# tonfengerqiguyisui/mapping-private

Measured on AMD Instinct MI355X. Metric: Mvoxels/s C3-HLAC + detections/s sliding-box, 256^3 grid, higher is better.
Workload: dtype u8 x u8 -> u32 (exact integer C3-HLAC), f32 search

## Files before the change

mapping-private_amd/csrc/c3h_internal.h:

```cpp
#pragma once
#include <hip/hip_runtime.h>

#include <cstdint>
#include <cstdlib>
#include <string>
#include <mutex>
#include <vector>

#include "../../include/c3hlac_mi355x.h"

namespace c3h {

constexpr uint32_t kOcc = 1u << 24;
constexpr uint32_t kEmptyKey = 0xffffffffu;
constexpr int kBlock = 256;
constexpr int kTileMax = 16;

constexpr float kNorm0 = 1 / 255.0;
constexpr float kNorm1 = 1 / 65025.0;
constexpr float kNorm117_1 = 1 / 845325.0;
constexpr float kNorm117_1Bin = 1 / 13.0;

template <class T>
struct DevBuf {
// ... 261 lines not shown
  const int32_t* types;
  int32_t* trans;
  int div_b[3], min_b[3], off[3], sb[3];
  float leaf, inv_leaf, inv_s;
  int hist1;
};
hipError_t nbr_build(NbrGrid& g, uint32_t* keys, uint32_t* keys2, uint32_t* idx, uint32_t* idx2, void* tmp,
                     size_t* tmp_bytes, hipStream_t s);
hipError_t launch_normals(const NbrGrid& g, float radius, const float vp[3], float4* out, hipStream_t s);
hipError_t launch_rsd(const NbrGrid& g, const float4* nrm, const float4* cent, int64_t nc, float max_dist,
                      float2* radii, int32_t* types, hipStream_t s);
hipError_t launch_grsd(const GrsdArgs& a, hipStream_t s);
hipError_t launch_grsd_feat(const int32_t* trans, int64_t H, float norm, float* out, int stride, hipStream_t s);
hipError_t launch_vosch_concat(const float* grsd, const float* c3, const int32_t* exist, int64_t H, float* out,
                               hipStream_t s);
hipError_t launch_pc2_convert(const void* data, uint32_t height, uint32_t width, uint32_t point_step,
                              uint32_t row_step, const int32_t off[4], int big, float* out, hipStream_t s);
hipError_t launch_exist_rule(const float* feat, int64_t H, int dim, int rule, int32_t* exist, hipStream_t s);

hipError_t launch_compress(const float* feat, int64_t H, int F, const float* axis_pt, int D,
                           int Dpad, const float* fmax, int fmax_len, float* G,
                           const int32_t* rows, const uint32_t* nrows, const int32_t* exist,
                           hipStream_t s);
hipError_t launch_masked_rows(const float* src, const int32_t* exist, int64_t H, int W, float* dst,
                              hipStream_t s);

struct ScoreLaunch {
  const float* G;
  const int32_t* exist;
  int D;
  int xn, yn, zn;
  int xr, yr, zr;
  int xe, ye, ze;
  int thr;
  const float* axis_q;
  const float* qt;
  int M, r, Opad;
  double* scores;
  ScorePartial* partials;
  int64_t order_base;
};
hipError_t launch_score(const ScoreLaunch& a, hipStream_t s);
bool score_fast_ok(int D, int r);
int64_t score_blocks(const ScoreLaunch& a);

struct ModeGeom {
  int64_t offset;
  int64_t P;
  int xe, ye, xr, yr, zr;
  int mode;
};
struct SparseSearch {
  const float* G;
  const int32_t* exist;
  int D, xn, yn, zn, thr;
  const float* qt;
  int M, r, Opad;
  int mpg;
  int group_loop;
  double* scores;
  ModeGeom md[6];
  int nmodes;
  int64_t pstart[7];
  int64_t order_base[6];
  long long* list;
  uint32_t* cnt;
  uint32_t epoch;
  int nframes;
  int64_t s_G, s_exist, s_scores, s_list, s_cnt, s_partials, s_lists;
  c3h_det* outs[kMaxBatch];
  ScorePartial* partials;
  uint32_t* done;
  c3h_det* lists;
  int clean;
  long long* prof;
  float* gbox = nullptr;
  int64_t s_gbox = 0;
  int score_mfma = 0;
  int skip_empty = 1;
  const _Float16* qt16 = nullptr;
  int Kq16 = 0;
  const int32_t* lim = nullptr;
  int sparse_scores = 0;
};
bool score_mfma_ok(int D);
struct SparseCompress {
  const float* feat;
  const float* PT;
  const float* fmax;
  float* G;
  const int32_t* rows;
  const uint32_t* nrows;
  int F, D, Dpad, fmax_len;
  int64_t H;
  int64_t s_feat, s_G, s_rows, s_nrows;
  const _Float16* PT16 = nullptr;
  int Fp16 = 0;
  const _Float16* feat16 = nullptr;
  const uint32_t* feat16_flag = nullptr;
  int f16s = 0;
};
bool compress_rows_ok(int F, int Dpad);
constexpr int64_t kBoxsumRows = 65536;
constexpr int64_t kCompressMfmaRows = 65536;
hipError_t launch_sparse_search(const SparseSearch& a, const SparseCompress* sc, hipStream_t s);
int64_t sparse_score_blocks(const SparseSearch& a);

struct ReplayMode {
  int64_t offset;
  int64_t P;
  int xe, ye;
  int mode;
};
struct ReplayModes {
  ReplayMode m[6];
  int n;
};
hipError_t launch_replay(const double* scores, const ReplayModes& modes, int M, int rank,
                         int r1, int r2, int r3, int clean, c3h_det* lists, c3h_det* out2,
                         hipStream_t s);

hipError_t launch_clean_lists(c3h_det* lists, int n, hipStream_t s);

struct TickParts {
  const C3Launch* occ = nullptr;
  const C3Launch* tile = nullptr;
  const SparseSearch* gate = nullptr;
  const SparseCompress* comp = nullptr;
  const SparseSearch* score = nullptr;
  DevBuf<long long>* prof = nullptr;
};
bool tick_ok(const C3Launch& l);
hipError_t launch_tick(const TickParts& p, hipStream_t s);
size_t c3hlac_lds_bytes(int tw_max, int list_max);
int64_t leaf_layout_blocks(int64_t nvox);

}

struct c3h_ctx {
  int device = 0;
  hipStream_t stream = nullptr;
  hipStream_t own_stream = nullptr;
  std::string err;

  c3h_ctx* parent = nullptr;
  std::vector<c3h_ctx*> lanes;
  std::vector<hipEvent_t> lane_ev;
  hipEvent_t fork_ev = nullptr;
  int nlanes = 3;
  int nbatch = 32;
  bool pipeline = true;
  uint64_t setup_version = 0;
  std::vector<float> h_axis_p, h_var, h_axis_q, h_fmax;

  bool have_grid = false;
  c3h_grid_info info{};
  c3h::DevBuf<uint32_t> grid;
  const uint32_t* grid_ptr = nullptr;
  c3h::DevBuf<float> pts;
  c3h::DevBuf<uint32_t> raw;
  c3h::DevBuf<float> dsbuf;
  c3h::DevBuf<float4> normals;
  bool normals_valid = false;
  c3h::NbrGrid nbr{};
  c3h::DevBuf<uint32_t> nkeys, nkeys2, nidx, nidx2, ncstart, ncend;
  c3h::DevBuf<uint8_t> ntmp;
// ... 159 lines not shown
```

mapping-private_amd/csrc/capi.hip:

```cpp
#include <algorithm>
#include <climits>
#include <cmath>
#include <cstdio>
#include <cstdlib>
#include <cstring>
#include <thread>

#include "c3h_internal.h"

using c3h::DevBuf;

namespace {

int fail(c3h_ctx* ctx, int code, const std::string& msg) {
  if (ctx) ctx->err = msg;
  return code;
}
int hip_fail(c3h_ctx* ctx, const char* what, hipError_t e) {
  return fail(ctx, C3H_ERR_HIP, std::string(what) + ": " + hipGetErrorString(e));
}

#define HIPCHK(expr)                                     \
  do {                                                   \
    hipError_t e_ = (expr);                              \
// ... 2078 lines not shown

struct PipeScope {
  c3h_ctx* ctx;
  hipStream_t saved[kPipeDepth - 1];
  explicit PipeScope(c3h_ctx* c) : ctx(c) {
    ctx->pipe_busy = true;
    for (int l = 0; l < kPipeDepth - 1 && l < (int)ctx->lanes.size(); ++l) {
      saved[l] = ctx->lanes[l]->stream;
      ctx->lanes[l]->stream = ctx->stream;
    }
  }
  ~PipeScope() {
    for (int l = 0; l < kPipeDepth - 1 && l < (int)ctx->lanes.size(); ++l) ctx->lanes[l]->stream = saved[l];
    ctx->pipe_busy = false;
  }
};

int pipe_tick(c3h_ctx* ctx, const c3h_ctx::PipeBatch* fresh) {
  c3h::TickParts tp;
  tp.prof = &ctx->prof;
  if (fresh && !fresh->stamped) tp.occ = &fresh->l;
  for (auto& b : ctx->pipe) {
    if (b.age == 1) tp.tile = &b.l;
    if (b.age == 2) {
      tp.gate = &b.q;
      tp.comp = &b.sc;
    }
    if (b.age == 3) tp.score = &b.q;
  }
  {
    Timed tm(ctx, 5, fresh ? fresh->nf : 0);
    hipError_t e = c3h::launch_tick(tp, ctx->stream);
    if (e != hipSuccess) return hip_fail(ctx, "launch_tick", e);
  }
  for (auto& b : ctx->pipe) {
    if (b.age == 2 && b.set) b.set->scores_layout = b.layout;
    if (b.age == 1 && b.fix) {
      hipError_t e = c3h::launch_point_fixup(b.fx, ctx->stream);
      if (e != hipSuccess) return hip_fail(ctx, "launch_point_fixup", e);
    }
  }
  std::vector<c3h_ctx::PipeBatch> next;
  for (auto& b : ctx->pipe)
    if (b.age < 3) {
      next.push_back(b);
      next.back().age++;
    }
  if (fresh) {
    next.push_back(*fresh);
    next.back().age = 1;
  }
  ctx->pipe.swap(next);
  return C3H_OK;
}

int pipe_flush(c3h_ctx* ctx) {
  if (ctx->pipe.empty()) return C3H_OK;
  PipeScope scope(ctx);
  while (!ctx->pipe.empty()) {
    int rc = pipe_tick(ctx, nullptr);
    if (rc != C3H_OK) {
      ctx->pipe.clear();
      return rc;
    }
  }
  return C3H_OK;
}

int pipe_quiesce(c3h_ctx* ctx) {
  if (ctx->pipe_busy || ctx->pipe.empty()) return C3H_OK;
  return pipe_flush(ctx);
}

int pipe_prepare(c3h_ctx* ctx, const uint32_t* const* grids, c3h_det* const* outs, int nb,
                 const c3h_ctx::PipeKey& k, const int32_t* lim, c3h_ctx::PipeBatch* fresh) {
  c3h_ctx* c = pipe_set(ctx, ctx->pipe_seq);
  c->capture = true;
  c->cap_c3_valid = c->cap_search_valid = false;
  int rc = c3h_set_grid(c, grids[0], k.div_b, k.min_b, k.leaf, 1);
  if (rc == C3H_OK) rc = extract_frames(c, grids, nb, &k.p, nullptr, nullptr);
  if (rc == C3H_OK) rc = search_frames(c, nb, k.range, k.thr, k.rotate, outs, 2);
  c->capture = false;
  c->cap_q.lim = lim;
  if (rc < 0) {
    if (c != ctx) ctx->err = c->err;
    return rc;
  }
  const bool fits = c->cap_c3_valid && c->cap_search_valid && c->cap_sparse_g && c->cap_argmax &&
                    c3h::tick_ok(c->cap_c3);
  if (!fits) {
    if (!ctx->pipe.empty()) return fail(ctx, C3H_ERR_STATE, "pipeline: internal: geometry changed");
    return 0;
  }
  c->nframes_feat = 1;
  *fresh = c3h_ctx::PipeBatch{c->cap_c3, c->cap_q, c->cap_sc, nb, 0};
  fresh->set = c;
  fresh->layout = c->cap_layout;
  return rc;
}

int pipe_commit(c3h_ctx* ctx, const c3h_ctx::PipeBatch& fresh, const c3h_ctx::PipeKey& k, int rc) {
  if (ctx->pipe.empty()) {
    for (int sidx = 0; sidx < kPipeDepth; ++sidx) {
      c3h_ctx* c = sidx == 0 ? ctx : (sidx - 1 < (int)ctx->lanes.size() ? ctx->lanes[sidx - 1] : nullptr);
      if (c && c->tileflags.p && c->tileflags.n >= 2)
        HIPCHK(hipMemsetAsync(c->tileflags.p, 0, 2 * sizeof(uint32_t), ctx->stream));
    }
  }
  int trc = pipe_tick(ctx, &fresh);
  if (trc != C3H_OK) return trc;
  ctx->pipe_seq++;
  ctx->pipe_key = k;
  ctx->pipe_nm = rc;
  return rc;
}

int pipe_push(c3h_ctx* ctx, const uint32_t* const* grids, c3h_det* const* outs, int nb,
              const c3h_ctx::PipeKey& k, const int32_t* lim = nullptr) {
  c3h_ctx::PipeBatch fresh{};
  const int rc = pipe_prepare(ctx, grids, outs, nb, k, lim, &fresh);
  if (rc <= 0) return rc;
  return pipe_commit(ctx, fresh, k, rc);
}

c3h_ctx::PipeKey pipe_key(c3h_ctx* ctx, const int32_t div_b[3], const int32_t min_b[3], float leaf,
                          const c3h_extract_params* p, const int32_t range[3], int32_t thr, int32_t rotate,
                          int B) {
  c3h_ctx::PipeKey k;
  memset(&k, 0, sizeof(k));
  memcpy(k.div_b, div_b, sizeof(k.div_b));
  memcpy(k.min_b, min_b, sizeof(k.min_b));
  k.leaf = leaf;
  k.p = *p;
  memcpy(k.range, range, sizeof(k.range));
  k.thr = thr;
  k.rotate = rotate ? 1 : 0;
  k.batch = B;
  k.rank = ctx->rank;
  k.setup_version = ctx->setup_version;
  return k;
}

bool pipelinable(const c3h_ctx* ctx) {
  return ctx->pipeline && ctx->rank == 1 && c3h::score_fast_ok(ctx->D, ctx->r);
}

int run_frames_pipelined(c3h_ctx* ctx, const uint32_t* const* d_grids, int32_t nframes,
                         const int32_t div_b[3], const int32_t min_b[3], float leaf,
                         const c3h_extract_params* p, const int32_t range[3], int32_t exist_threshold,
                         int32_t rotate, c3h_det* d_out, int B, bool drain) {
  const size_t per_frame = (size_t)std::max(ctx->M, 1) * ctx->rank;
  const int nchunks = (nframes + B - 1) / B;
  int rc = ensure_lanes(ctx, kPipeDepth - 1);
  if (rc != C3H_OK) return rc;
  const c3h_ctx::PipeKey k = pipe_key(ctx, div_b, min_b, leaf, p, range, exist_threshold, rotate, B);
  if (!ctx->pipe.empty() && memcmp(&k, &ctx->pipe_key, sizeof(k)) != 0) {
    rc = pipe_flush(ctx);
    if (rc != C3H_OK) return rc;
  }
  PipeScope scope(ctx);
  if (drain && ctx->pipe.empty())
    ctx->pipe_seq = (uint64_t)((kPipeDepth - (nchunks - 1) % kPipeDepth) % kPipeDepth);
  int nm = 0;
  for (int ch = 0; ch < nchunks; ++ch) {
    const uint32_t* grids[c3h::kMaxBatch];
    c3h_det* outs[c3h::kMaxBatch];
// ... 686 lines not shown
```

mapping-private_amd/csrc/pipeline.hip:

```cpp
#include <algorithm>
#include <climits>
#include <cstdio>
#include <cstdlib>
#include <cstring>
#include <vector>

#include "c3hlac_dev.h"
#include "search_dev.h"

namespace c3h {
namespace {

struct TickArgs {
  int n_score, n_cg, n_tile, n_occ;
  SparseSearch sq;
  int s_gx, s_groups;
  SparseSearch gq;
  CompressRows cr;
  int g_ngate, g_ncomp;
  int comp_mfma;
  KArgs ka;
  int t_grid;
  OccArgs oa;
  int o_grid;
  int order;
  int xcd;
  long long* prof;
};

__device__ __forceinline__ int tick_canonical_block(const TickArgs& t) {
  const int n[4] = {t.n_occ, t.n_tile, t.n_cg, t.n_score};
  int b = blockIdx.x;
  for (int i = 0; i < 4; ++i) {
    const int r = (t.order >> (4 * i)) & 15;
    if (b < n[r]) {
      for (int k = 0; k < r; ++k) b += n[k];
      return b;
    }
    b -= n[r];
  }
  return b;
}

#ifndef C3H_TICK_PRIO_OCC
#define C3H_TICK_PRIO_OCC 3
#endif
#ifndef C3H_TICK_PRIO_TILE
#define C3H_TICK_PRIO_TILE 0
#endif
#ifndef C3H_TICK_PRIO_CG
#define C3H_TICK_PRIO_CG 0
#endif
#ifndef C3H_TICK_PRIO_SCORE
#define C3H_TICK_PRIO_SCORE 0
#endif
#define C3H_SETPRIO(p) \
  if constexpr ((p) > 0) __builtin_amdgcn_s_setprio(p)

__device__ __forceinline__ void role_frame(int b, int g, bool xcd, int& f, int& local) {
  if (xcd) {
    const int q = b >> 3, k = q / g;
    f = (b & 7) + 8 * k;
    local = q - k * g;
  } else {
    f = b / g;
    local = b - f * g;
  }
}

__device__ __forceinline__ void tick_roles(const TickArgs& t, uint32_t* tick_smem) {
  int b = t.order == 0x3210 ? (int)blockIdx.x : tick_canonical_block(t);
  int f, r;
  if (b < t.n_occ) {
    C3H_SETPRIO(C3H_TICK_PRIO_OCC);
    role_frame(b, t.o_grid, t.xcd & 1, f, r);
    occupancy_bits_body<true>(t.oa, r, f, t.o_grid, tick_smem);
    return;
  }
  b -= t.n_occ;
  if (b < t.n_tile) {
    C3H_SETPRIO(C3H_TICK_PRIO_TILE);
    role_frame(b, t.t_grid, t.xcd & 2, f, r);
    if (t.ka.wave117) c3hlac_wave117_body(t.ka, r, f, t.t_grid, tick_smem);
    else c3hlac_tile_body(t.ka, r, f, t.t_grid, tick_smem);
    return;
  }
  b -= t.n_tile;
  if (b < t.n_cg) {
    C3H_SETPRIO(C3H_TICK_PRIO_CG);
    role_frame(b, t.g_ngate + t.g_ncomp, t.xcd & 4, f, r);
    if (r < t.g_ngate) gate_body(t.gq, r, f);
    else if (t.comp_mfma) compress_f32t_body(t.cr, r - t.g_ngate, t.g_ncomp, f, reinterpret_cast<float*>(tick_smem));
    else compress_rows_body(t.cr, r - t.g_ngate, t.g_ncomp, f, reinterpret_cast<float*>(tick_smem));
    return;
  }
  b -= t.n_cg;
  C3H_SETPRIO(C3H_TICK_PRIO_SCORE);
  role_frame(b, t.s_gx * t.s_groups, t.xcd & 8, f, r);
  score_list_body(t.sq, r % t.s_gx, r / t.s_gx, f, t.s_gx, t.s_groups, reinterpret_cast<float*>(tick_smem));
}

#ifndef C3H_TICK_MINW
#define C3H_TICK_MINW 4
#endif
__global__ __launch_bounds__(kBlock, C3H_TICK_MINW) void c3h_tick_kernel(TickArgs t) {
  extern __shared__ __attribute__((aligned(16))) uint32_t tick_smem[];
  if (t.prof && threadIdx.x == 0) t.prof[2 * blockIdx.x] = (long long)wall_clock64();
  tick_roles(t, tick_smem);
  if (t.prof) {
    __syncthreads();
    if (threadIdx.x == 0) t.prof[2 * blockIdx.x + 1] = (long long)wall_clock64();
  }
}

void tick_prof_dump(const TickArgs& t, long long* d_prof, int total, hipStream_t s) {
  std::vector<long long> v((size_t)2 * total);
  if (hipMemcpyAsync(v.data(), d_prof, v.size() * 8, hipMemcpyDeviceToHost, s) != hipSuccess) return;
  if (hipStreamSynchronize(s) != hipSuccess) return;
  FILE* fp = fopen(diag_env("C3H_TICK_PROF"), "a");
  if (!fp) return;
  long long t0 = LLONG_MAX;
  for (int b = 0; b < total; ++b) t0 = std::min(t0, v[2 * b]);
  const int n[4] = {t.n_occ, t.n_tile, t.n_cg, t.n_score};
  const char* names[4] = {"occ", "tile", "cg", "score"};
  int b0 = 0;
  fprintf(fp, "tick");
  for (int i = 0; i < 4; ++i) {
    const int r = (t.order >> (4 * i)) & 15;
    if (n[r]) {
      long long smin = LLONG_MAX, smax = 0, emax = 0;
      double dsum = 0;
      for (int b = b0; b < b0 + n[r]; ++b) {
        smin = std::min(smin, v[2 * b]);
        smax = std::max(smax, v[2 * b]);
        emax = std::max(emax, v[2 * b + 1]);
        dsum += v[2 * b + 1] - v[2 * b];
      }
      fprintf(fp, " %s[n=%d start=%.1f..%.1f end=%.1f mean=%.1f]", names[r], n[r], (smin - t0) * 0.01,
              (smax - t0) * 0.01, (emax - t0) * 0.01, dsum / n[r] * 0.01);
      if (r == 0 && t.o_grid > 0) {
        double fmin = 1e30, fmax = 0, wmax = 0;
        const int nfr = n[r] / t.o_grid;
        std::vector<long long> lo(nfr, LLONG_MAX), hi(nfr, 0);
        for (int b = 0; b < n[r]; ++b) {
          const int f = (t.xcd & 1) ? (b & 7) + 8 * ((b >> 3) / t.o_grid) : b / t.o_grid;
          lo[f] = std::min(lo[f], v[2 * (b0 + b) + 1]);
          hi[f] = std::max(hi[f], v[2 * (b0 + b) + 1]);
        }
        for (int f = 0; f < nfr; ++f) {
          fmin = std::min(fmin, (hi[f] - t0) * 0.01);
          fmax = std::max(fmax, (hi[f] - t0) * 0.01);
          wmax = std::max(wmax, (hi[f] - lo[f]) * 0.01);
        }
        fprintf(fp, " occ_frame_end[%.1f..%.1f within<=%.1f]", fmin, fmax, wmax);
        std::vector<double> ends;
        for (int b = b0; b < b0 + n[r]; ++b) ends.push_back((v[2 * b + 1] - t0) * 0.01);
        std::sort(ends.begin(), ends.end());
        fprintf(fp, " occ_end_p10/50/90[%.1f %.1f %.1f]", ends[ends.size() / 10], ends[ends.size() / 2],
                ends[ends.size() * 9 / 10]);
      }
    }
    b0 += n[r];
  }
  fprintf(fp, "\n");
  fclose(fp);
}

int env_int(const char* name, int dflt) {
  const char* v = diag_env(name);
  return v && *v ? atoi(v) : dflt;
}

}

bool tick_ok(const C3Launch& l) {
  const C3Args c = build_c3_args(l);
  return c.bits && c.ax && !l.atomic && l.prof == nullptr && l.debug == 0;
}

hipError_t launch_tick(const TickParts& p, hipStream_t s) {
  TickArgs t{};
  size_t lds = 16;
#ifndef C3H_TICK_ORDER_DEFAULT
#define C3H_TICK_ORDER_DEFAULT 0x2130
#endif
  t.order = p.occ ? C3H_TICK_ORDER_DEFAULT : 0x3210;
  if (const char* o = diag_env("C3H_TICK_ORDER"))
    if (strlen(o) == 4) {
      t.order = 0;
      for (int i = 0; i < 4; ++i) t.order |= (o[i] - '0') << (4 * i);
    }
  if (p.score) {
    const SparseSearch& a = *p.score;
    t.sq = a;
    t.s_gx = (int)std::max<int64_t>(1, std::min<int64_t>(sparse_score_blocks(a), env_int("C3H_TICK_SCORE", 16)));
    t.s_groups = (a.M + a.mpg - 1) / a.mpg;
#ifndef C3H_TICK_GROUP_LOOP
#define C3H_TICK_GROUP_LOOP 1
#endif
    if (C3H_TICK_GROUP_LOOP && t.s_groups > 1 && a.D * kOC >= kFP * (kOC + 1)) {
      t.sq.group_loop = 1;
      t.s_groups = 1;
    }
    lds = std::max(lds, score_list_lds_bytes(a.D, a.mpg));
    t.n_score = t.s_gx * t.s_groups * a.nframes;
  }
  if (p.gate) {
    const SparseSearch& a = *p.gate;
    const SparseCompress& sc = *p.comp;
    t.gq = a;
    t.cr = CompressRows{sc.feat, sc.PT, sc.fmax, sc.G, sc.rows, sc.nrows, sc.F, sc.D, sc.Dpad,
                        sc.fmax_len, sc.s_feat, sc.s_G, sc.s_rows, sc.s_nrows};
    t.g_ngate = (int)((a.pstart[a.nmodes] + kBlock - 1) / kBlock);
#ifndef C3H_TICK_COMP_MFMA
#define C3H_TICK_COMP_MFMA 1
#endif
    t.comp_mfma = env_int("C3H_TICK_COMP_MFMA", C3H_TICK_COMP_MFMA) && sc.Dpad <= 128 ? 1 : 0;
    if (t.comp_mfma) {
      t.g_ncomp = (int)std::max<int64_t>(1, std::min<int64_t>((sc.H + kCR - 1) / kCR, env_int("C3H_TICK_COMP", 16)));
      lds = std::max(lds, kTLds);
    } else {
      t.g_ncomp = (int)std::max<int64_t>(1, std::min<int64_t>((sc.H + kRR - 1) / kRR, env_int("C3H_TICK_COMP", 32)));
      lds = std::max(lds, compress_rows_lds_bytes(sc.Dpad));
    }
    t.n_cg = (t.g_ngate + t.g_ncomp) * a.nframes;
  }
  if (p.tile) {
    const C3Args c = build_c3_args(*p.tile);
    t.ka = c.ka;
    const int work = std::max(1, std::min(c.tgrid - c.ka.zblocks, env_int("C3H_TICK_TILE", 48)));
    t.ka.zblocks = std::min(c.ka.zblocks, env_int("C3H_TICK_ZERO", 8));
    t.t_grid = t.ka.zblocks + work;
    t.n_tile = t.t_grid * c.nframes;
    lds = std::max(lds, c.tile_lds);
  }
  if (p.occ) {
    const C3Args c = build_c3_args(*p.occ);
    t.oa = c.oa;
    t.o_grid = std::max(1, std::min(c.g1, env_int("C3H_TICK_OCC", std::max(1, 256 / std::max(1, c.nframes)))));
    t.n_occ = t.o_grid * c.nframes;
    lds = std::max(lds, c.occ_lds);
#ifndef C3H_TICK_STEAL_DIV
#define C3H_TICK_STEAL_DIV 16
#endif
#ifndef C3H_TICK_STEAL_UNIT
#define C3H_TICK_STEAL_UNIT 8
#endif
    const int64_t n4 = (int64_t)c.oa.gx * c.oa.gy * c.oa.gz / 4;
    const bool rowwave = occ_rowwave(c.oa.gx, c.ax);
    const int64_t nch = occ_nchunks(n4, occ_depth(rowwave));
    const int div = env_int("C3H_TICK_STEAL_DIV", C3H_TICK_STEAL_DIV);
    const int unit = env_int("C3H_TICK_STEAL_UNIT", C3H_TICK_STEAL_UNIT);
    const OccSteal st = rowwave ? occ_steal_plan(nch, c.nframes, div, unit) : OccSteal{0, 0, 0};
    if (st.unit > 0) {
      t.oa.steal_from = st.from;
      t.oa.steal_unit = st.unit;
      t.oa.steal_units = st.units;
      t.oa.nframes = c.nframes;
      t.oa.steal_wgs = t.n_occ;
    }
  }
  if (const char* m = diag_env("C3H_TICK_ROLES")) {
    const int mask = atoi(m);
    if (!(mask & 1)) t.n_score = 0;
    if (!(mask & 2)) t.n_cg = 0;
    if (!(mask & 4)) t.n_tile = 0;
    if (!(mask & 8)) t.n_occ = 0;
  }
  const int total = t.n_score + t.n_cg + t.n_tile + t.n_occ;
  if (total == 0) return hipSuccess;
#ifndef C3H_TICK_XCD
#define C3H_TICK_XCD 15
#endif
  t.xcd = 0;
  {
    const int nb[4] = {t.n_occ, t.n_tile, t.n_cg, t.n_score};
    const int per[4] = {t.o_grid, t.t_grid, t.g_ngate + t.g_ncomp, t.s_gx * t.s_groups};
    int base = 0;
    for (int i = 0; i < 4; ++i) {
      const int r = (t.order >> (4 * i)) & 15;
      if (nb[r] > 0 && per[r] > 0 && base % 8 == 0 && (nb[r] / per[r]) % 8 == 0) t.xcd |= 1 << r;
      base += nb[r];
    }
// ... 20 lines not shown
```

mapping-private_amd/csrc/search_dev.h:

```cpp
#pragma once
#include "c3h_internal.h"

namespace c3h {

constexpr int kRR = 16, kRK = 32;
constexpr int kRS = kRK + 1;
constexpr int kCompressGridCap = 128;
__host__ __device__ inline size_t compress_rows_lds_bytes(int Dpad) {
  return sizeof(float) * ((size_t)kRK * Dpad + (size_t)kRR * kRS);
}

struct CompressRows {
  const float* feat;
  const float* PT;
  const float* fmax;
  float* G;
  const int32_t* rows;
  const uint32_t* nrows;
  int F, D, Dpad, fmax_len;
  int64_t s_feat, s_G, s_rows, s_nrows;
  int64_t H = 0;
  const _Float16* feat16 = nullptr;
  const uint32_t* feat16_flag = nullptr;
  int f16s = 0;
// ... 463 lines not shown
  }
  const unsigned long long m = __ballot(pass);
  if (m) {
    uint32_t base = 0;
    if (lane == 0) base = atomicAdd(&fcnt[a.epoch & 1], (uint32_t)__popcll(m));
    base = __shfl(base, 0, 64);
    if (pass) flist[base + __popcll(m & ((1ull << lane) - 1))] = entry;
  }
}

__device__ __forceinline__ void boxsum_body(const SparseSearch& a, int64_t e, int64_t f) {
  const int D4 = a.D >> 2;
  const int64_t g = e / D4;
  const int d4 = (int)(e - g * D4);
  if (g >= a.pstart[a.nmodes]) return;
  const int mi = find_mode(a, g);
  const ModeGeom& md = a.md[mi];
  const int64_t p = g - a.pstart[mi];
  const int64_t xye = (int64_t)md.xe * md.ye;
  const int x = (int)(p % md.xe), y = (int)((p / md.xe) % md.ye), z = (int)(p / xye);
  const int xyn = a.xn * a.yn;
  const int h = z * xyn + y * a.xn + x;
  const int32_t* __restrict__ fexist = a.exist + f * a.s_exist;
  const float4* G4 = reinterpret_cast<const float4*>(a.G + f * a.s_G);
  float4 s = make_float4(0.f, 0.f, 0.f, 0.f);
  for (int dz = 0; dz < md.zr; ++dz)
    for (int dy = 0; dy < md.yr; ++dy)
      for (int dx = 0; dx < md.xr; ++dx) {
        const int hh = h + dz * xyn + dy * a.xn + dx;
        if (!a.skip_empty || fexist[hh] != 0) {
          const float4 v = G4[(int64_t)hh * D4 + d4];
          s.x += v.x;
          s.y += v.y;
          s.z += v.z;
          s.w += v.w;
        }
      }
  reinterpret_cast<float4*>(a.gbox + f * a.s_gbox)[g * D4 + d4] = s;
}

__device__ void argmax_finalize(const SparseSearch& a, const ScorePartial* partials, c3h_det* lists,
                                c3h_det* out, int nparts, int model_base = 0, int model_stride = kBlock / 64) {
  const int lane = threadIdx.x & 63, w = threadIdx.x >> 6;
  for (int m = model_base + w; m < a.M; m += model_stride) {
    double best = -2.0;
    long long bo = -1;
    for (int i = lane; i < nparts; i += 64) {
      const ScorePartial* q = partials + (int64_t)i * a.M + m;
      const long long qo = __hip_atomic_load(&q->order, __ATOMIC_RELAXED, __HIP_MEMORY_SCOPE_AGENT);
      const double qs = __hip_atomic_load(&q->score, __ATOMIC_RELAXED, __HIP_MEMORY_SCOPE_AGENT);
      if (qo >= 0 && (qs > best || (qs == best && qo < bo))) {
        best = qs;
        bo = qo;
      }
    }
#pragma unroll
    for (int o = 32; o > 0; o >>= 1) {
      const double os = __shfl_xor(best, o, 64);
      const long long oo = __shfl_xor(bo, o, 64);
      if (oo >= 0 && (os > best || (os == best && (bo < 0 || oo < bo)))) {
        best = os;
        bo = oo;
      }
    }
    if (lane == 0) {
      c3h_det e = lists[m];
      if (a.clean) {
        e.score = 0.0;
        e.x = e.y = e.z = 0;
        if (a.clean == 2) e.mode = 0;
      }
      if (bo >= 0 && best > e.score) {
        const int mi = (int)(bo >> 40);
        const int64_t p = bo & ((1ll << 40) - 1);
        const ModeGeom& md = a.md[mi];
        e.score = best;
        e.x = (int)(p % md.xe);
        e.y = (int)((p / md.xe) % md.ye);
        e.z = (int)(p / ((int64_t)md.xe * md.ye));
        e.mode = md.mode;
      }
      lists[m] = e;
      if (out) out[m] = e;
    }
  }
}

__host__ __device__ inline size_t score_list_lds_bytes(int D, int mpg) {
  const size_t region = ((size_t)D * kFP > (size_t)kFP * (kOC + 1) ? (size_t)D * kFP : (size_t)kFP * (kOC + 1)) +
                        (size_t)D * kOC;
  return sizeof(float) * (region + kFP) + sizeof(int) * 4 * kFP + sizeof(long long) * kFP +
         sizeof(double) * kFP * mpg + 16 + 16;
}

__device__ __forceinline__ void score_list_body(const SparseSearch& b, int bx, int by, int fz_, int gdx, int gdy,
                                                float* ssm) {
  const SparseSearch& a = b;
  const int64_t fz = fz_;
  const float* __restrict__ fG = b.G + fz * b.s_G;
  const int32_t* __restrict__ fexist = b.exist + fz * b.s_exist;
  double* __restrict__ fscores = b.scores + fz * b.s_scores;
  const long long* __restrict__ flist = b.list + fz * b.s_list;
  const uint32_t* fcnt = b.cnt + fz * b.s_cnt;
  uint32_t* fdone = b.done + fz * b.s_cnt;
  ScorePartial* fpart = b.partials ? b.partials + fz * b.s_partials : nullptr;
  c3h_det* flists = b.lists ? b.lists + fz * b.s_lists : nullptr;
  c3h_det* fout = b.outs[fz];
  long long* fprof = fz ? nullptr : b.prof;
  const int D = a.D, D4 = a.D >> 2, Qs = a.Opad;
#define C3H_SPROF(k) \
  if (fprof && threadIdx.x == 0 && by == 0) fprof[bx * 8 + (k)] = (long long)wall_clock64()
  C3H_SPROF(0);
  const int tid = threadIdx.x;
  const int64_t ptot = a.pstart[a.nmodes];
  long long en_first = -1;
  if (tid < kFP) en_first = flist[min((int64_t)bx * kFP + tid, ptot - 1)];
  const int ngl = a.group_loop ? (a.M + a.mpg - 1) / a.mpg : 1;
  const int fts = max(D * kFP, kFP * (kOC + 1));
  auto issue_window = [&](int grp) {
    constexpr int kQW = 160 * kOC / kBlock;
    const int g0 = grp * a.mpg, g1 = min(a.M, g0 + a.mpg);
    const int row0 = g0 * a.r, oc = ((g1 - g0) * a.r + 15) & ~15;
    float* qwl = ssm + fts;
    const int wave = tid >> 6;
#pragma unroll 4
    for (int j = 0; j < kQW; ++j) {
      const int e = j * kBlock + tid, d = e / oc, o = e - d * oc;
      if (j * kBlock >= D * oc) break;
      if (e < D * oc)
        __builtin_amdgcn_global_load_lds(a.qt + (int64_t)d * Qs + row0 + o, qwl + j * kBlock + wave * 64, 4, 0, 0);
    }
  };
  issue_window(by);
  const int n = (int)fcnt[a.epoch & 1];
  const int nch = (n + kFP - 1) / kFP;
  if (bx >= nch) {
    __asm__ volatile("s_waitcnt vmcnt(0)" ::: "memory");
    if (n == 0 && flists && bx == 0 && by == 0) argmax_finalize(a, fpart, flists, fout, 0);
    return;
  }
  float* fT = ssm;
  float* qw = ssm + fts;
  float* qv = a.group_loop ? qw : ssm;
  float* ffv = qw + D * kOC;
  int* gate = reinterpret_cast<int*>(ffv + kFP);
  int* hrow = gate + kFP;
  int* rng = hrow + kFP;
  long long* ent = reinterpret_cast<long long*>(rng + kFP + (kFP & 1));
  double* bsc = reinterpret_cast<double*>(ent + kFP);
  const int xyn = a.xn * a.yn;
  for (int ch = bx; ch < nch; ch += gdx) {
    const int64_t e0 = (int64_t)ch * kFP;
    if (tid < kFP) {
      const int64_t e = e0 + tid;
      int ok = 0, h = 0, rr = 0;
      long long en = -1;
      if (e < n) {
        en = ch == bx ? en_first : flist[e];
        const int mi = (int)(en >> 40);
        const int64_t p = en & ((1ll << 40) - 1);
        const ModeGeom& md = a.md[mi];
        const int64_t xye = (int64_t)md.xe * md.ye;
        const int x = (int)(p % md.xe), y = (int)((p / md.xe) % md.ye), z = (int)(p / xye);
        h = z * xyn + y * a.xn + x;
        rr = md.xr | (md.yr << 10) | (md.zr << 20);
        ok = 1;
      }
      gate[tid] = ok;
      hrow[tid] = h;
      rng[tid] = rr;
      ent[tid] = en;
    }
    lds_barrier();
    C3H_SPROF(1);
    if (b.gbox) {
      const float4* B4 = reinterpret_cast<const float4*>(b.gbox + fz * b.s_gbox);
      for (int e = tid; e < kFP * D4; e += kBlock) {
        const int pp = e & (kFP - 1), d4 = e / kFP;
        float4 v = make_float4(0.f, 0.f, 0.f, 0.f);
        if (gate[pp]) {
          const long long en = ent[pp];
          v = B4[(a.pstart[(int)(en >> 40)] + (en & ((1ll << 40) - 1))) * D4 + d4];
        }
        fT[(4 * d4 + 0) * kFP + pp] = v.x;
        fT[(4 * d4 + 1) * kFP + pp] = v.y;
        fT[(4 * d4 + 2) * kFP + pp] = v.z;
        fT[(4 * d4 + 3) * kFP + pp] = v.w;
      }
    } else {
      const int pp = tid & (kFP - 1), dg = tid / kFP;
      constexpr int kDG = kBlock / kFP;
      const bool ok = gate[pp];
      const int h = hrow[pp], rr = rng[pp];
      const int xr = rr & 1023, yr = (rr >> 10) & 1023, zr = rr >> 20;
      const int ncell = ok ? xr * yr * zr : 0;
      const float4* G4 = reinterpret_cast<const float4*>(fG);
      constexpr int kSlots = 4;
      constexpr int kCB = C3H_SCORE_CB;
      float4 s[kSlots];
#pragma unroll
      for (int q = 0; q < kSlots; ++q) s[q] = make_float4(0.f, 0.f, 0.f, 0.f);
      for (int d4b = 0; d4b < D4; d4b += kSlots * kDG) {
        for (int c0 = 0; c0 < ncell; c0 += kCB) {
          float4 g[kCB][kSlots];
          bool lv[kCB];
#pragma unroll
          for (int k = 0; k < kCB; ++k) {
            const int c = c0 + k;
            const int dx = c % xr, dy = (c / xr) % yr, dz = c / (xr * yr);
            const int hh = h + dz * xyn + dy * a.xn + dx;
            lv[k] = c < ncell && (!a.skip_empty || fexist[c < ncell ? hh : h] != 0);
#pragma unroll
            for (int q = 0; q < kSlots; ++q) {
              const int d4 = d4b + dg + q * kDG;
              g[k][q] = (c < ncell && d4 < D4) ? G4[(int64_t)hh * D4 + d4] : make_float4(0.f, 0.f, 0.f, 0.f);
            }
          }
#pragma unroll
          for (int k = 0; k < kCB; ++k)
#pragma unroll
            for (int q = 0; q < kSlots; ++q)
              if (lv[k]) {
                s[q].x += g[k][q].x;
                s[q].y += g[k][q].y;
                s[q].z += g[k][q].z;
                s[q].w += g[k][q].w;
              }
        }
#pragma unroll
        for (int q = 0; q < kSlots; ++q) {
          const int d4 = d4b + dg + q * kDG;
          if (d4 < D4) {
            fT[(4 * d4 + 0) * kFP + pp] = s[q].x;
            fT[(4 * d4 + 1) * kFP + pp] = s[q].y;
            fT[(4 * d4 + 2) * kFP + pp] = s[q].z;
            fT[(4 * d4 + 3) * kFP + pp] = s[q].w;
          }
          s[q] = make_float4(0.f, 0.f, 0.f, 0.f);
        }
      }
    }
    __asm__ volatile("s_waitcnt vmcnt(0)" ::: "memory");
    lds_barrier();
    C3H_SPROF(2);
    if (tid < kFP) {
      float s = 0.0f;
      for (int d = 0; d < D; ++d) s = __builtin_fmaf(fT[d * kFP + tid], fT[d * kFP + tid], s);
      ffv[tid] = s;
    }
    for (int gi = 0; gi < ngl; ++gi) {
      const int grp = by + gi;
      const int m0 = grp * a.mpg, m1 = min(a.M, m0 + a.mpg);
      const int oc = ((m1 - m0) * a.r + 15) & ~15;
      if (a.group_loop && (gi > 0 || ch != bx)) {
        lds_barrier();
        issue_window(grp);
        __asm__ volatile("s_waitcnt vmcnt(0)" ::: "memory");
        lds_barrier();
      }
      const int tp = tid & 15, to = tid >> 4;
      const bool active = 4 * to < oc;
      float acc[2][4];
#pragma unroll
      for (int i = 0; i < 2; ++i)
#pragma unroll
        for (int q = 0; q < 4; ++q) acc[i][q] = 0.0f;
      if (active) {
#pragma unroll 4
        for (int d = 0; d < D; ++d) {
          const float2 f = *reinterpret_cast<const float2*>(&fT[d * kFP + 2 * tp]);
          const float4 q = *reinterpret_cast<const float4*>(&qw[d * oc + 4 * to]);
          acc[0][0] = __builtin_fmaf(f.x, q.x, acc[0][0]);
          acc[0][1] = __builtin_fmaf(f.x, q.y, acc[0][1]);
          acc[0][2] = __builtin_fmaf(f.x, q.z, acc[0][2]);
          acc[0][3] = __builtin_fmaf(f.x, q.w, acc[0][3]);
          acc[1][0] = __builtin_fmaf(f.y, q.x, acc[1][0]);
          acc[1][1] = __builtin_fmaf(f.y, q.y, acc[1][1]);
          acc[1][2] = __builtin_fmaf(f.y, q.z, acc[1][2]);
          acc[1][3] = __builtin_fmaf(f.y, q.w, acc[1][3]);
        }
      }
      lds_barrier();
      C3H_SPROF(3);
      if (active) {
#pragma unroll
        for (int i = 0; i < 2; ++i)
#pragma unroll
          for (int q = 0; q < 4; ++q) qv[(2 * tp + i) * (kOC + 1) + 4 * to + q] = acc[i][q];
      }
      lds_barrier();
      const int nm = m1 - m0;
      for (int e = tid; e < kFP * nm; e += kBlock) {
        const int mm = e / kFP, pp = e - mm * kFP;
        double sc = -2.0;
        if (gate[pp]) {
          float q2 = 0.0f;
          const float* q = qv + pp * (kOC + 1) + mm * a.r;
#pragma unroll 4
          for (int i = 0; i < a.r; ++i) q2 = __builtin_fmaf(q[i], q[i], q2);
          sc = sqrt((double)q2) / sqrt((double)ffv[pp]);
          const long long en = ent[pp];
          const ModeGeom& md = a.md[(int)(en >> 40)];
          fscores[md.offset + (int64_t)(m0 + mm) * md.P + (en & ((1ll << 40) - 1))] = sc;
        }
        bsc[e] = sc;
      }
      C3H_SPROF(4);
      if (fpart) {
        lds_barrier();
        for (int mm = tid; mm < nm; mm += kBlock) {
          double best = -2.0;
          long long bo = -1;
          for (int pp = 0; pp < kFP; ++pp) {
            if (!gate[pp]) continue;
            const double sc = bsc[mm * kFP + pp];
            const long long en = ent[pp];
            const long long o = a.order_base[(int)(en >> 40)] + (en & ((1ll << 40) - 1));
            if (sc > best || (sc == best && o < bo)) {
              best = sc;
              bo = o;
            }
          }
          ScorePartial* q = fpart + (int64_t)ch * a.M + m0 + mm;
          if (flists) {
            __hip_atomic_store(&q->score, best, __ATOMIC_RELAXED, __HIP_MEMORY_SCOPE_AGENT);
            __hip_atomic_store(&q->order, bo, __ATOMIC_RELAXED, __HIP_MEMORY_SCOPE_AGENT);
          } else {
            *q = ScorePartial{best, bo};
          }
        }
      }
    }
    lds_barrier();
  }
  if (fpart && flists) {
    int& s_last = *reinterpret_cast<int*>(reinterpret_cast<char*>(ssm) + score_list_lds_bytes(D, a.mpg) - 16);
    __asm__ volatile("s_waitcnt vmcnt(0)" ::: "memory");
    lds_barrier();
    if (tid == 0) {
      const uint32_t total = (uint32_t)min(nch, gdx) * gdy;
      s_last = atomicAdd(&fdone[a.epoch & 1], 1u) == total - 1;
    }
    lds_barrier();
    if (s_last) argmax_finalize(a, fpart, flists, fout, nch);
  }
  C3H_SPROF(7);
}

}
```

Measured before the change: 1.316 million.

## Add MFMA-based score body to fused tick kernel replacing group loop

Adds a score path inside the persistent tick kernel that gathers box-summed feature rows once per chunk, then computes the projections for many models at once with 32x32x2 f32 MFMA. Query columns are prefetched from global memory in blocks of eight, and the per-model scores and argmax partials are written from LDS. The path is on by default whenever there is more than one model group, and replaces the scalar group-loop scoring with matrix-core work. The shared gather code is factored into a helper. The risk is extra LDS traffic, register pressure and barrier cost, plus scalar f32 MFMA precision behaviour.

```diff
diff --git a/mapping-private_amd/csrc/c3h_internal.h b/mapping-private_amd/csrc/c3h_internal.h
--- a/mapping-private_amd/csrc/c3h_internal.h
+++ b/mapping-private_amd/csrc/c3h_internal.h
@@ -367,6 +367,7 @@
   int Kq16 = 0;
   const int32_t* lim = nullptr;
   int sparse_scores = 0;
+  int score_engine = 0;
 };
 bool score_mfma_ok(int D);
 struct SparseCompress {
diff --git a/mapping-private_amd/csrc/capi.hip b/mapping-private_amd/csrc/capi.hip
--- a/mapping-private_amd/csrc/capi.hip
+++ b/mapping-private_amd/csrc/capi.hip
@@ -2184,6 +2184,7 @@
   if (rc == C3H_OK) rc = search_frames(c, nb, k.range, k.thr, k.rotate, outs, 2);
   c->capture = false;
   c->cap_q.lim = lim;
+  c->cap_q.score_engine = ctx->score_engine;
   if (rc < 0) {
     if (c != ctx) ctx->err = c->err;
     return rc;
diff --git a/mapping-private_amd/csrc/pipeline.hip b/mapping-private_amd/csrc/pipeline.hip
--- a/mapping-private_amd/csrc/pipeline.hip
+++ b/mapping-private_amd/csrc/pipeline.hip
@@ -15,6 +15,7 @@
   int n_score, n_cg, n_tile, n_occ;
   SparseSearch sq;
   int s_gx, s_groups;
+  int s_mpp;
   SparseSearch gq;
   CompressRows cr;
   int g_ngate, g_ncomp;
@@ -97,7 +98,8 @@
   b -= t.n_cg;
   C3H_SETPRIO(C3H_TICK_PRIO_SCORE);
   role_frame(b, t.s_gx * t.s_groups, t.xcd & 8, f, r);
-  score_list_body(t.sq, r % t.s_gx, r / t.s_gx, f, t.s_gx, t.s_groups, reinterpret_cast<float*>(tick_smem));
+  if (t.s_mpp > 0) score_tick_mfma_body(t.sq, r, f, t.s_gx, t.s_mpp, reinterpret_cast<float*>(tick_smem));
+  else score_list_body(t.sq, r % t.s_gx, r / t.s_gx, f, t.s_gx, t.s_groups, reinterpret_cast<float*>(tick_smem));
 }
 
 #ifndef C3H_TICK_MINW
@@ -198,7 +200,14 @@
 #ifndef C3H_TICK_GROUP_LOOP
 #define C3H_TICK_GROUP_LOOP 1
 #endif
-    if (C3H_TICK_GROUP_LOOP && t.s_groups > 1 && a.D * kOC >= kFP * (kOC + 1)) {
+#ifndef C3H_TICK_SCORE_MFMA
+#define C3H_TICK_SCORE_MFMA 1
+#endif
+    if (env_int("C3H_TICK_SCORE_MFMA", C3H_TICK_SCORE_MFMA) && a.score_engine != 1 &&
+        (t.s_groups > 1 || a.score_engine == 2)) {
+      t.s_mpp = score_tick_mpp(a.D, a.M, a.r, a.mpg);
+      t.s_groups = 1;
+    } else if (C3H_TICK_GROUP_LOOP && t.s_groups > 1 && a.D * kOC >= kFP * (kOC + 1)) {
       t.sq.group_loop = 1;
       t.s_groups = 1;
     }
diff --git a/mapping-private_amd/csrc/search_dev.h b/mapping-private_amd/csrc/search_dev.h
--- a/mapping-private_amd/csrc/search_dev.h
+++ b/mapping-private_amd/csrc/search_dev.h
@@ -569,6 +569,63 @@
       }
       lists[m] = e;
       if (out) out[m] = e;
+    }
+  }
+}
+
+__device__ __forceinline__ void score_gather_rows(const SparseSearch& a, const float* __restrict__ fG,
+                                                  const int32_t* __restrict__ fexist, const int* gate,
+                                                  const int* hrow, const int* rng, float* fT) {
+  const int tid = threadIdx.x, D4 = a.D >> 2, xyn = a.xn * a.yn;
+  const int pp = tid & (kFP - 1), dg = tid / kFP;
+  constexpr int kDG = kBlock / kFP;
+  const bool ok = gate[pp];
+  const int h = hrow[pp], rr = rng[pp];
+  const int xr = rr & 1023, yr = (rr >> 10) & 1023, zr = rr >> 20;
+  const int ncell = ok ? xr * yr * zr : 0;
+  const float4* G4 = reinterpret_cast<const float4*>(fG);
+  constexpr int kSlots = 4;
+  constexpr int kCB = C3H_SCORE_CB;
+  float4 s[kSlots];
+#pragma unroll
+  for (int q = 0; q < kSlots; ++q) s[q] = make_float4(0.f, 0.f, 0.f, 0.f);
+  for (int d4b = 0; d4b < D4; d4b += kSlots * kDG) {
+    for (int c0 = 0; c0 < ncell; c0 += kCB) {
+      float4 g[kCB][kSlots];
+      bool lv[kCB];
+#pragma unroll
+      for (int k = 0; k < kCB; ++k) {
+        const int c = c0 + k;
+        const int dx = c % xr, dy = (c / xr) % yr, dz = c / (xr * yr);
+        const int hh = h + dz * xyn + dy * a.xn + dx;
+        lv[k] = c < ncell && (!a.skip_empty || fexist[c < ncell ? hh : h] != 0);
+#pragma unroll
+        for (int q = 0; q < kSlots; ++q) {
+          const int d4 = d4b + dg + q * kDG;
+          g[k][q] = (c < ncell && d4 < D4) ? G4[(int64_t)hh * D4 + d4] : make_float4(0.f, 0.f, 0.f, 0.f);
+        }
+      }
+#pragma unroll
+      for (int k = 0; k < kCB; ++k)
+#pragma unroll
+        for (int q = 0; q < kSlots; ++q)
+          if (lv[k]) {
+            s[q].x += g[k][q].x;
+            s[q].y += g[k][q].y;
+            s[q].z += g[k][q].z;
+            s[q].w += g[k][q].w;
+          }
+    }
+#pragma unroll
+    for (int q = 0; q < kSlots; ++q) {
+      const int d4 = d4b + dg + q * kDG;
+      if (d4 < D4) {
+        fT[(4 * d4 + 0) * kFP + pp] = s[q].x;
+        fT[(4 * d4 + 1) * kFP + pp] = s[q].y;
+        fT[(4 * d4 + 2) * kFP + pp] = s[q].z;
+        fT[(4 * d4 + 3) * kFP + pp] = s[q].w;
+      }
+      s[q] = make_float4(0.f, 0.f, 0.f, 0.f);
     }
   }
 }
@@ -675,57 +732,7 @@
         fT[(4 * d4 + 3) * kFP + pp] = v.w;
       }
     } else {
-      const int pp = tid & (kFP - 1), dg = tid / kFP;
-      constexpr int kDG = kBlock / kFP;
-      const bool ok = gate[pp];
-      const int h = hrow[pp], rr = rng[pp];
-      const int xr = rr & 1023, yr = (rr >> 10) & 1023, zr = rr >> 20;
-      const int ncell = ok ? xr * yr * zr : 0;
-      const float4* G4 = reinterpret_cast<const float4*>(fG);
-      constexpr int kSlots = 4;
-      constexpr int kCB = C3H_SCORE_CB;
-      float4 s[kSlots];
-#pragma unroll
-      for (int q = 0; q < kSlots; ++q) s[q] = make_float4(0.f, 0.f, 0.f, 0.f);
-      for (int d4b = 0; d4b < D4; d4b += kSlots * kDG) {
-        for (int c0 = 0; c0 < ncell; c0 += kCB) {
-          float4 g[kCB][kSlots];
-          bool lv[kCB];
-#pragma unroll
-          for (int k = 0; k < kCB; ++k) {
-            const int c = c0 + k;
-            const int dx = c % xr, dy = (c / xr) % yr, dz = c / (xr * yr);
-            const int hh = h + dz * xyn + dy * a.xn + dx;
-            lv[k] = c < ncell && (!a.skip_empty || fexist[c < ncell ? hh : h] != 0);
-#pragma unroll
-            for (int q = 0; q < kSlots; ++q) {
-              const int d4 = d4b + dg + q * kDG;
-              g[k][q] = (c < ncell && d4 < D4) ? G4[(int64_t)hh * D4 + d4] : make_float4(0.f, 0.f, 0.f, 0.f);
-            }
-          }
-#pragma unroll
-          for (int k = 0; k < kCB; ++k)
-#pragma unroll
-            for (int q = 0; q < kSlots; ++q)
-              if (lv[k]) {
-                s[q].x += g[k][q].x;
-                s[q].y += g[k][q].y;
-                s[q].z += g[k][q].z;
-                s[q].w += g[k][q].w;
-              }
-        }
-#pragma unroll
-        for (int q = 0; q < kSlots; ++q) {
-          const int d4 = d4b + dg + q * kDG;
-          if (d4 < D4) {
-            fT[(4 * d4 + 0) * kFP + pp] = s[q].x;
-            fT[(4 * d4 + 1) * kFP + pp] = s[q].y;
-            fT[(4 * d4 + 2) * kFP + pp] = s[q].z;
-            fT[(4 * d4 + 3) * kFP + pp] = s[q].w;
-          }
-          s[q] = make_float4(0.f, 0.f, 0.f, 0.f);
-        }
-      }
+      score_gather_rows(a, fG, fexist, gate, hrow, rng, fT);
     }
     __asm__ volatile("s_waitcnt vmcnt(0)" ::: "memory");
     lds_barrier();
@@ -834,4 +841,198 @@
   C3H_SPROF(7);
 }
 
-}
+constexpr int kTickQS = kFP + 1;
+constexpr int kTickPF = 8;
+__host__ __device__ inline int score_tick_tiles(int models, int r) { return (models * r + 31) / 32; }
+__host__ __device__ inline size_t score_tick_lds_bytes(int D, int M, int r, int mpp) {
+  const size_t ft = (size_t)D * kFP, qv = (size_t)kTickQS * 32 * score_tick_tiles(mpp, r);
+  const size_t region = mpp >= M ? (ft > qv ? ft : qv) : ft + qv;
+  return sizeof(float) * (region + kFP) + sizeof(int) * 4 * kFP + sizeof(long long) * kFP +
+         sizeof(double) * kFP * mpp + 16 + 16;
+}
+__host__ __device__ inline int score_tick_mpp(int D, int M, int r, int mpg) {
+  const size_t budget = score_list_lds_bytes(D, mpg);
+  int mpp = M;
+  while (mpp > 1 && (score_tick_tiles(mpp, r) > 8 || score_tick_lds_bytes(D, M, r, mpp) > budget)) --mpp;
+  return mpp;
+}
+
+__device__ __forceinline__ void score_tick_mfma_body(const SparseSearch& b, int bx, int fz_, int gdx, int mpp,
+                                                     float* ssm) {
+  const SparseSearch& a = b;
+  const int64_t fz = fz_;
+  const float* __restrict__ fG = b.G + fz * b.s_G;
+  const int32_t* __restrict__ fexist = b.exist + fz * b.s_exist;
+  double* __restrict__ fscores = b.scores + fz * b.s_scores;
+  const long long* __restrict__ flist = b.list + fz * b.s_list;
+  const uint32_t* fcnt = b.cnt + fz * b.s_cnt;
+  uint32_t* fdone = b.done + fz * b.s_cnt;
+  ScorePartial* fpart = b.partials ? b.partials + fz * b.s_partials : nullptr;
+  c3h_det* flists = b.lists ? b.lists + fz * b.s_lists : nullptr;
+  c3h_det* fout = b.outs[fz];
+  long long* fprof = fz ? nullptr : b.prof;
+  constexpr int by = 0;
+  const int D = a.D, Qs = a.Opad;
+  C3H_SPROF(0);
+  const int tid = threadIdx.x, lane = tid & 63, wave = tid >> 6, hk = lane >> 5, l32 = lane & 31;
+  const int64_t ptot = a.pstart[a.nmodes];
+  long long en_first = -1;
+  if (tid < kFP) en_first = flist[min((int64_t)bx * kFP + tid, ptot - 1)];
+  const int n = (int)fcnt[a.epoch & 1];
+  const int nch = (n + kFP - 1) / kFP;
+  if (bx >= nch) {
+    if (n == 0 && flists && bx == 0) argmax_finalize(a, fpart, flists, fout, 0);
+    return;
+  }
+  const int nqv = kTickQS * 32 * score_tick_tiles(mpp, a.r);
+  const bool one_pass = mpp >= a.M;
+  float* fT = ssm;
+  float* qv = one_pass ? ssm : ssm + D * kFP;
+  float* ffv = ssm + (one_pass ? max(D * kFP, nqv) : D * kFP + nqv);
+  int* gate = reinterpret_cast<int*>(ffv + kFP);
+  int* hrow = gate + kFP;
+  int* rng = hrow + kFP;
+  long long* ent = reinterpret_cast<long long*>(rng + kFP + (kFP & 1));
+  double* bsc = reinterpret_cast<double*>(ent + kFP);
+  const int xyn = a.xn * a.yn;
+  const int KP = D >> 1;
+  for (int ch = bx; ch < nch; ch += gdx) {
+    const int64_t e0 = (int64_t)ch * kFP;
+    if (tid < kFP) {
+      const int64_t e = e0 + tid;
+      int ok = 0, h = 0, rr = 0;
+      long long en = -1;
+      if (e < n) {
+        en = ch == bx ? en_first : flist[e];
+        const int mi = (int)(en >> 40);
+        const int64_t p = en & ((1ll << 40) - 1);
+        const ModeGeom& md = a.md[mi];
+        const int64_t xye = (int64_t)md.xe * md.ye;
+        const int x = (int)(p % md.xe), y = (int)((p / md.xe) % md.ye), z = (int)(p / xye);
+        h = z * xyn + y * a.xn + x;
+        rr = md.xr | (md.yr << 10) | (md.zr << 20);
+        ok = 1;
+      }
+      gate[tid] = ok;
+      hrow[tid] = h;
+      rng[tid] = rr;
+      ent[tid] = en;
+    }
+    lds_barrier();
+    C3H_SPROF(1);
+    score_gather_rows(a, fG, fexist, gate, hrow, rng, fT);
+    lds_barrier();
+    C3H_SPROF(2);
+    if (tid >= kBlock - 64 && lane < kFP) {
+      float s = 0.0f;
+      for (int d = 0; d < D; ++d) s = __builtin_fmaf(fT[d * kFP + lane], fT[d * kFP + lane], s);
+      ffv[lane] = s;
+    }
+    for (int m0 = 0; m0 < a.M; m0 += mpp) {
+      const int m1 = min(a.M, m0 + mpp), nm = m1 - m0;
+      const int c0 = m0 * a.r, ncol = nm * a.r, ntile = (ncol + 31) >> 5;
+      const int t = wave;
+      const bool one = t < ntile, two = t + 4 < ntile;
+      mf_f32x16 acc0, acc1;
+#pragma unroll
+      for (int q = 0; q < 16; ++q) acc0[q] = acc1[q] = 0.0f;
+      if (one) {
+        const uint32_t v0 = (uint32_t)(hk * Qs + min(c0 + 32 * t + l32, Qs - 1));
+        const uint32_t v1 = two ? (uint32_t)(hk * Qs + min(c0 + 32 * (t + 4) + l32, Qs - 1)) : v0;
+        float bc[2][kTickPF], bn[2][kTickPF];
+        auto load_b = [&](float (&v)[2][kTickPF], int j0) {
+#pragma unroll
+          for (int jj = 0; jj < kTickPF; ++jj) {
+            const float* __restrict__ rowp = a.qt + (int64_t)min(2 * (j0 + jj), D - 2) * Qs;
+            v[0][jj] = rowp[v0];
+            v[1][jj] = rowp[v1];
+          }
+        };
+        load_b(bc, 0);
+        for (int j0 = 0; j0 < KP; j0 += kTickPF) {
+          if (j0 + kTickPF < KP) load_b(bn, j0 + kTickPF);
+#pragma unroll
+          for (int jj = 0; jj < kTickPF; ++jj) {
+            if (j0 + jj < KP) {
+              const float av = fT[(2 * (j0 + jj) + hk) * kFP + l32];
+              acc0 = __builtin_amdgcn_mfma_f32_32x32x2f32(av, bc[0][jj], acc0, 0, 0, 0);
+              if (two) acc1 = __builtin_amdgcn_mfma_f32_32x32x2f32(av, bc[1][jj], acc1, 0, 0, 0);
+            }
+          }
+#pragma unroll
+          for (int jj = 0; jj < kTickPF; ++jj) {
+            bc[0][jj] = bn[0][jj];
+            bc[1][jj] = bn[1][jj];
+          }
+        }
+      }
+      lds_barrier();
+      C3H_SPROF(3);
+      if (one) {
+#pragma unroll
+        for (int q = 0; q < 16; ++q) qv[(32 * t + l32) * kTickQS + 4 * hk + (q & 3) + 8 * (q >> 2)] = acc0[q];
+      }
+      if (two) {
+#pragma unroll
+        for (int q = 0; q < 16; ++q)
+          qv[(32 * (t + 4) + l32) * kTickQS + 4 * hk + (q & 3) + 8 * (q >> 2)] = acc1[q];
+      }
+      lds_barrier();
+      for (int e = tid; e < kFP * nm; e += kBlock) {
+        const int mm = e / kFP, pp = e - mm * kFP;
+        double sc = -2.0;
+        if (gate[pp]) {
+          float q2 = 0.0f;
+          const float* q = qv + mm * a.r * kTickQS + pp;
+#pragma unroll 4
+          for (int i = 0; i < a.r; ++i) q2 = __builtin_fmaf(q[i * kTickQS], q[i * kTickQS], q2);
+          sc = sqrt((double)q2) / sqrt((double)ffv[pp]);
+          const long long en = ent[pp];
+          const ModeGeom& md = a.md[(int)(en >> 40)];
+          fscores[md.offset + (int64_t)(m0 + mm) * md.P + (en & ((1ll << 40) - 1))] = sc;
+        }
+        bsc[e] = sc;
+      }
+      C3H_SPROF(4);
+      if (fpart) {
+        lds_barrier();
+        for (int mm = tid; mm < nm; mm += kBlock) {
+          double best = -2.0;
+          long long bo = -1;
+          for (int pp = 0; pp < kFP; ++pp) {
+            if (!gate[pp]) continue;
+            const double sc = bsc[mm * kFP + pp];
+            const long long en = ent[pp];
+            const long long o = a.order_base[(int)(en >> 40)] + (en & ((1ll << 40) - 1));
+            if (sc > best || (sc == best && o < bo)) {
+              best = sc;
+              bo = o;
+            }
+          }
+          ScorePartial* q = fpart + (int64_t)ch * a.M + m0 + mm;
+          if (flists) {
+            __hip_atomic_store(&q->score, best, __ATOMIC_RELAXED, __HIP_MEMORY_SCOPE_AGENT);
+            __hip_atomic_store(&q->order, bo, __ATOMIC_RELAXED, __HIP_MEMORY_SCOPE_AGENT);
+          } else {
+            *q = ScorePartial{best, bo};
+          }
+        }
+      }
+    }
+    lds_barrier();
+  }
+  if (fpart && flists) {
+    int& s_last = *reinterpret_cast<int*>(reinterpret_cast<char*>(ssm) + score_list_lds_bytes(D, a.mpg) - 16);
+    __asm__ volatile("s_waitcnt vmcnt(0)" ::: "memory");
+    lds_barrier();
+    if (tid == 0) {
+      const uint32_t total = (uint32_t)min(nch, gdx);
+      s_last = atomicAdd(&fdone[a.epoch & 1], 1u) == total - 1;
+    }
+    lds_barrier();
+    if (s_last) argmax_finalize(a, fpart, flists, fout, nch);
+  }
+  C3H_SPROF(7);
+}
+
+}
```

Result: faster. 1.344 million (median of 6 runs) (+2.1%).
